# kunpengcompute/media

Measured on AMD Instinct MI355X. Metric: encoded fps @1080p I420 baseline-profile, 1/2/4/8 MI355X vs OpenH264 CPU, higher is better.
Workload: dtype u8

## Files before the change

### media_amd/csrc/k_me.h

```cpp
#pragma once
#include "dev_common.h"
#include "mc_filters.h"

namespace h264 {

enum { ME_R = 16, ME_AP = 4, ME_WS = 16 + 2 * ME_R + 2 * ME_AP, ME_WDW = ME_WS / 4, ME_GS = 18, ME_GP = 20, ME_PLS = ME_GS * ME_GP };

__device__ __forceinline__ void qpel_taps(int fx, int fy, int& o0, int& o1)
{
    const int PL = ME_PLS;
    const int G = 0, B = PL, H = 2 * PL, J = 3 * PL, R = 1, D = ME_GP;
    switch (fy * 4 + fx) {
        case 0: o0 = G; o1 = G; break;
        case 1: o0 = G; o1 = B; break;
        case 2: o0 = B; o1 = B; break;
        case 3: o0 = G + R; o1 = B; break;
        case 4: o0 = G; o1 = H; break;
        case 5: o0 = B; o1 = H; break;
        case 6: o0 = B; o1 = J; break;
        case 7: o0 = B; o1 = H + R; break;
        case 8: o0 = H; o1 = H; break;
        case 9: o0 = H; o1 = J; break;
        case 10: o0 = J; o1 = J; break;
        case 11: o0 = H + R; o1 = J; break;
        case 12: o0 = G + D; o1 = H; break;
        case 13: o0 = B + D; o1 = H; break;
        case 14: o0 = B + D; o1 = J; break;
        default: o0 = B + D; o1 = H + R; break;
    }
}


__device__ __forceinline__ uint32_t chroma_pred4(const uint8_t* cp, int cs2, int chh, int x0, int y0, int fx, int fy)
{
    const uint8_t* r0 = cp + (size_t)clip3(0, chh - 1, y0) * cs2;
    const uint8_t* r1 = cp + (size_t)clip3(0, chh - 1, y0 + 1) * cs2;
    uint32_t A, B, C, D;
    if (x0 >= 0 && (x0 & ~3) + 8 <= cs2) {
        const int xa = x0 & ~3, sh = x0 & 3;
        const uint32_t a0 = *(const uint32_t*)(r0 + xa), a1 = *(const uint32_t*)(r0 + xa + 4);
        const uint32_t c0 = *(const uint32_t*)(r1 + xa), c1 = *(const uint32_t*)(r1 + xa + 4);
        A = __builtin_amdgcn_alignbyte(a1, a0, sh); B = sh == 3 ? a1 : __builtin_amdgcn_alignbyte(a1, a0, sh + 1);
        C = __builtin_amdgcn_alignbyte(c1, c0, sh); D = sh == 3 ? c1 : __builtin_amdgcn_alignbyte(c1, c0, sh + 1);
    } else {
        A = B = C = D = 0;
#pragma unroll
        for (int k = 0; k < 4; k++) {
            const int xa = clip3(0, cs2 - 1, x0 + k), xb = clip3(0, cs2 - 1, x0 + k + 1);
            A |= (uint32_t)r0[xa] << (8 * k); B |= (uint32_t)r0[xb] << (8 * k);
            C |= (uint32_t)r1[xa] << (8 * k); D |= (uint32_t)r1[xb] << (8 * k);
        }
    }
    if ((fx | fy) == 0) return A;
    const int w00 = (8 - fx) * (8 - fy), w10 = fx * (8 - fy), w01 = (8 - fx) * fy, w11 = fx * fy;
    uint32_t o = 0;
#pragma unroll
    for (int k = 0; k < 4; k++)
        o |= (uint32_t)((w00 * byte_of(A, k) + w10 * byte_of(B, k) + w01 * byte_of(C, k) + w11 * byte_of(D, k) + 32) >> 6) << (8 * k);
    return o;
}

#ifndef ME_WAVES_MIN
#define ME_WAVES_MIN 6
#endif
template <bool IND = false>
__global__ __launch_bounds__(64) __attribute__((amdgpu_waves_per_eu(ME_WAVES_MIN, 8))) void k_me(FrameParams P0)
{
    if (AB_PRIO_ME) __builtin_amdgcn_s_setprio(AB_PRIO_ME);
    const FrameParams P = batch_view<IND>(P0, blockIdx.y);
    const int lane = threadIdx.x;
    const int mbi = P.band.row0 * P.mbw + xcd_mb_index(blockIdx.x, P.mbw * P.band.rows), my = P.mbdiv.row(mbi), mx = mbi - my * P.mbw;
    const int bx = 16 * mx, by = 16 * my;

    __shared__ __attribute__((aligned(16))) uint32_t s_win[ME_WS * ME_WDW];
    __shared__ __attribute__((aligned(16))) uint8_t s_src[256];
    __shared__ __attribute__((aligned(16))) uint8_t s_srcc[128];
    __shared__ __attribute__((aligned(16))) uint32_t s_ytab[32];
    __shared__ __attribute__((aligned(16))) uint8_t s_refc[128];
    enum { ME_B1_BYTES = (ME_GS + 5) * ME_GP * 2, ME_PL_BYTES = 4 * ME_PLS + 16 };
    enum { ME_TASKCAP = 760 };
    __shared__ __attribute__((aligned(16))) uint8_t s_scr[4 * ME_TASKCAP > ME_B1_BYTES + ME_PL_BYTES ? 4 * ME_TASKCAP : ME_B1_BYTES + ME_PL_BYTES];
    __shared__ unsigned s_ntask;
    uint32_t* const s_task = (uint32_t*)s_scr;
    int16_t* const s_b1 = (int16_t*)s_scr;
    uint8_t* const s_pl = s_scr + ME_B1_BYTES;

    const int pmw = __builtin_amdgcn_readfirstlane(P.rf == 0 ? *(const int*)(P.mb + mbi) : P.pmv[mbi]);
    if (P.rf == 0 && P.rf_last > 0 && lane == 0) P.pmv[mbi] = pmw;
    const int pmx = (int)(int16_t)(pmw & 0xFFFF), pmy = pmw >> 16;
    load_src_mb(P, mx, my, s_src, s_srcc, lane);
    const int rf = P.rf;
    unsigned prev_total = 0xFFFFFFFFu;
    if (rf > 0) {
        prev_total = (unsigned)__builtin_amdgcn_readfirstlane((int)P.me_total[mbi]);
        if (prev_total == 0u) return;
    }
    const uint8_t* const RY = P.ref[0];
    const uint8_t* const RU = P.ref[1];
    const uint8_t* const RV = P.ref[2];
    {
        const int wx0 = bx - ME_R - ME_AP, wy0 = by - ME_R - ME_AP;
        const bool inside = wx0 >= 0 && wx0 + 64 <= P.cw && wy0 >= 0 && wy0 + ME_WS <= P.ch;
        if (inside) {
            const int c = lane & 15, rg = lane >> 4;
            const uint8_t* rp = RY + (size_t)(wy0 + rg) * P.cw + wx0 + 4 * c;
            const size_t step = (size_t)4 * P.cw;
            uint32_t v[14];
#pragma unroll
            for (int t = 0; t < 14; t++) v[t] = *(const uint32_t*)(rp + t * step);
            if (c < ME_WDW)
#pragma unroll
                for (int t = 0; t < 14; t++) s_win[(rg + 4 * t) * ME_WDW + c] = v[t];
        } else {
            const bool interior = wx0 >= 0 && bx + 16 + ME_R + ME_AP <= P.cw;
            uint32_t v[13];
#pragma unroll
            for (int t = 0; t < 13; t++) {
                const int i = lane + 64 * t;
                const int row = i / ME_WDW, dw = i - row * ME_WDW;
                const int gy = clip3(0, P.ch - 1, wy0 + row);
                const int gx = wx0 + dw * 4;
                const uint8_t* rp = RY + (size_t)gy * P.cw;
                v[t] = 0;
                if (i < ME_WS * ME_WDW) {
                    if (interior) v[t] = *(const uint32_t*)(rp + gx);
                    else {
#pragma unroll
                        for (int k = 0; k < 4; k++) v[t] |= (uint32_t)rp[clip3(0, P.cw - 1, gx + k)] << (8 * k);
                    }
                }
            }
#pragma unroll
            for (int t = 0; t < 13; t++)
                if (lane + 64 * t < ME_WS * ME_WDW) s_win[lane + 64 * t] = v[t];
        }
    }
    if (rf == 0 && lane < 32) {
        const int pl = lane >> 4, row = (lane >> 1) & 7, xs = (lane & 1) * 4;
        *(uint32_t*)(s_refc + pl * 64 + row * 8 + xs) =
            *(const uint32_t*)((pl ? P.ref[2] : P.ref[1]) + (size_t)(8 * my + row) * (P.cw / 2) + 8 * mx + xs);
    }
    __syncthreads();
    const uint8_t* winb = (const uint8_t*)s_win;

    if (rf == 0) {
        typedef unsigned short pk16 __attribute__((ext_vector_type(2)));
        const int r = lane & 3, b4 = lane >> 2;
        const int cplz = lane >> 4, cyz = ((lane >> 3) & 1) * 4 + r, cxz = ((lane >> 2) & 1) * 4;
        const uint32_t sy = *(const uint32_t*)(s_src + ((b4 >> 2) * 4 + r) * 16 + (b4 & 3) * 4);
        const uint32_t sc = lane < 32 ? *(const uint32_t*)(s_srcc + cplz * 64 + cyz * 8 + cxz) : 0u;
        const uint32_t one = 0x00010001u;
        const pk16 sA = __builtin_bit_cast(pk16, (r & 1) ? 0xFFFFFFFFu : one);
        const pk16 mA = __builtin_bit_cast(pk16, r == 1 ? 2u * one : one);
        const pk16 mB = __builtin_bit_cast(pk16, r < 2 ? one : (r == 2 ? 0xFFFFFFFFu : 0xFFFEFFFEu));
        const uint32_t t0 = (uint32_t)(P.qy.thr_inter[0] - 1) | ((uint32_t)(P.qc.thr_inter[0] - 1) << 16);
        const uint32_t t1 = (uint32_t)(P.qy.thr_inter[1] - 1) | ((uint32_t)(P.qc.thr_inter[1] - 1) << 16);
        const uint32_t t2 = (uint32_t)(P.qy.thr_inter[2] - 1) | ((uint32_t)(P.qc.thr_inter[2] - 1) << 16);
        const pk16 th_even = __builtin_bit_cast(pk16, (r & 1) ? t2 : t0), th_odd = __builtin_bit_cast(pk16, (r & 1) ? t1 : t2);
        auto quantises_to_nothing = [&](uint32_t ry, uint32_t rc) -> bool {
            pk16 d[4];
#pragma unroll
            for (int k = 0; k < 4; k++) {
                const uint32_t sel = 0x0c040c00u + 0x00010001u * k;
                d[k] = __builtin_bit_cast(pk16, __builtin_amdgcn_perm(sc, sy, sel)) - __builtin_bit_cast(pk16, __builtin_amdgcn_perm(rc, ry, sel));
            }
            {
                const pk16 s0 = d[0] + d[3], s1 = d[1] + d[2], d0 = d[0] - d[3], d1 = d[1] - d[2];
                d[0] = s0 + s1; d[1] = d0 + d0 + d1; d[2] = s0 - s1; d[3] = d0 - d1 - d1;
            }
            uint32_t over = 0;
            int dc = 0;
#pragma unroll
            for (int c = 0; c < 4; c++) {
                if (c == 1 && __ballot(over != 0) != 0ull) return false;
                const pk16 q0 = __builtin_bit_cast(pk16, quad_bcast<0>(__builtin_bit_cast(int, d[c])));
                const pk16 q1 = __builtin_bit_cast(pk16, quad_bcast<1>(__builtin_bit_cast(int, d[c])));
                const pk16 q2 = __builtin_bit_cast(pk16, quad_bcast<2>(__builtin_bit_cast(int, d[c])));
                const pk16 q3 = __builtin_bit_cast(pk16, quad_bcast<3>(__builtin_bit_cast(int, d[c])));
                const pk16 A = q0 + sA * q3, B = q1 + sA * q2;
                const pk16 w = mA * A + mB * B;
                if (c == 0) dc = (int)(short)w.y;
                typedef short spk16 __attribute__((ext_vector_type(2)));
                const spk16 ws = __builtin_bit_cast(spk16, w);
                const pk16 aw = __builtin_bit_cast(pk16, __builtin_elementwise_max(ws, -ws));
                uint32_t ov = __builtin_bit_cast(uint32_t, __builtin_elementwise_sub_sat(aw, (c & 1) ? th_odd : th_even));
                if (c == 0 && r == 0) ov &= 0xFFFFu;
                over |= ov;
            }
            bool dcnz = false;
#pragma unroll
            for (int pl = 0; pl < 2; pl++) {
                const int d0 = __builtin_amdgcn_readlane(dc, pl * 16), d1 = __builtin_amdgcn_readlane(dc, pl * 16 + 4);
                const int d2 = __builtin_amdgcn_readlane(dc, pl * 16 + 8), d3 = __builtin_amdgcn_readlane(dc, pl * 16 + 12);
                const int t = P.qc.thr_dc_inter;
                dcnz |= iabs(d0 + d1 + d2 + d3) >= t || iabs(d0 - d1 + d2 - d3) >= t || iabs(d0 + d1 - d2 - d3) >= t || iabs(d0 - d1 - d2 + d3) >= t;
            }
            return !dcnz && __ballot(over != 0) == 0ull;
        };
        auto luma_sad = [&](uint32_t ry) -> unsigned {
            const int s = row_sum16_dpp((int)__builtin_amdgcn_sad_u8(sy, ry, 0u));
            return (unsigned)(__builtin_amdgcn_readlane(s, 0) + __builtin_amdgcn_readlane(s, 16) + __builtin_amdgcn_readlane(s, 32) + __builtin_amdgcn_readlane(s, 48));
        };
        auto settle = [&](int vx, int vy, uint32_t ry, uint32_t rc) {
            *(uint32_t*)(P.rec[0] + (size_t)(by + (b4 >> 2) * 4 + r) * P.cw + bx + (b4 & 3) * 4) = ry;
            if (lane < 32) *(uint32_t*)((cplz ? P.rec[2] : P.rec[1]) + (size_t)(8 * my + cyz) * (P.cw / 2) + 8 * mx + cxz) = rc;
            if (lane == 0) {
                uint4* m = (uint4*)(P.mb + mbi);
                m[0] = make_uint4(((uint32_t)vx & 0xFFFFu) | ((uint32_t)vy << 16), (uint32_t)MB_P16 | (0x80u << 8), 0u, 0u);
                m[1] = make_uint4(0u, 0u, 0u, 0u);
                const uint32_t v = ((uint32_t)vx & 0xFFFFu) | ((uint32_t)vy << 16);
                *(uint4*)(P.mvq + (size_t)mbi * 8) = make_uint4(v, v, v, v);
                P.me_cost[mbi] = 0;
                P.me_total[mbi] = 0u;
            }
        };
        {
            const uint32_t ry = s_win[(ME_R + ME_AP + (b4 >> 2) * 4 + r) * ME_WDW + (ME_R + ME_AP) / 4 + (b4 & 3)];
            const uint32_t rc = lane < 32 ? *(const uint32_t*)(s_refc + cplz * 64 + cyz * 8 + cxz) : 0u;
            if (luma_sad(ry) < (unsigned)P.sad_nz && quantises_to_nothing(ry, rc)) { settle(0, 0, ry, rc); return; }
        }
        const int rvx = ((pmx + 2) >> 2) * 4, rvy = ((pmy + 2) >> 2) * 4;
        if ((rvx | rvy) != 0) {
            const uint32_t ry = lds_ld4(winb, (ME_R + ME_AP + (b4 >> 2) * 4 + r + (rvy >> 2)) * ME_WS + ME_R + ME_AP + (b4 & 3) * 4 + (rvx >> 2));
            uint32_t rc = 0;
            if (lane < 32) rc = chroma_pred4(cplz ? P.ref[2] : P.ref[1], P.cw / 2, P.ch / 2, 8 * mx + cxz + (rvx >> 3), 8 * my + cyz + (rvy >> 3), rvx & 7, rvy & 7);
            if (luma_sad(ry) < (unsigned)P.sad_nz && quantises_to_nothing(ry, rc)) { settle(rvx, rvy, ry, rc); return; }
        }
    }

    unsigned best = 0xFFFFFFFFu;
    bool seeded = false;
    if (P.search == 1) {
        const int sx = (pmx + 2) >> 2, sy = (pmy + 2) >> 2;
        if (sx >= -ME_R && sx < ME_R && sy >= -ME_R && sy < ME_R) {
            const int g = lane >> 4, j = lane & 15;
            const int dyc = sy - 1 + (g < 3 ? g : 0);
            const uint4 sv = *(const uint4*)(s_src + 16 * j);
            const int ob = (ME_R + ME_AP + dyc + j) * ME_WS + ME_R + ME_AP + sx - 1;
            int sad3[3];
#pragma unroll
            for (int k = 0; k < 3; k++) {
                uint32_t a = __builtin_amdgcn_sad_u8(lds_ld4(winb, ob + k), sv.x, 0u);
                a = __builtin_amdgcn_sad_u8(lds_ld4(winb, ob + k + 4), sv.y, a);
                a = __builtin_amdgcn_sad_u8(lds_ld4(winb, ob + k + 8), sv.z, a);
                a = __builtin_amdgcn_sad_u8(lds_ld4(winb, ob + k + 12), sv.w, a);
                sad3[k] = row_sum16_dpp((int)a);
            }
            unsigned ckey = 0, nmin = 0xFFFFFFFFu;
#pragma unroll
            for (int gy = 0; gy < 3; gy++)
#pragma unroll
                for (int k = 0; k < 3; k++) {
                    const int dx = sx - 1 + k, dy = sy - 1 + gy;
                    const unsigned sad = (unsigned)__builtin_amdgcn_readlane(sad3[k], 16 * gy);
                    const unsigned key = ((sad + (unsigned)(P.lambda * (se_len(4 * dx - pmx) + se_len(4 * dy - pmy)))) << 10) | (unsigned)(((dy + ME_R) << 5) | (dx + ME_R));
                    const bool inr = dx >= -ME_R && dx < ME_R && dy >= -ME_R && dy < ME_R;
                    if (gy == 1 && k == 1) ckey = key;
                    else if (inr && key < nmin) nmin = key;
                }
            if (ckey < nmin) { best = ckey; seeded = true; }
        }
    }

    if (!seeded) {
        const int dxi = lane & 31, half = lane >> 5;
        const int col = dxi + ME_AP, cdw = col >> 2, sh = col & 3;
        if (lane < 32) s_ytab[lane] = ((uint32_t)__mul24(P.lambda, se_len(4 * (lane - ME_R) - pmy)) << 10) | ((uint32_t)lane << 5);
        uint32_t srow[16][4];
        const uint8_t* sp0 = P.src + (size_t)by * P.w + bx;
        if (bx + 16 <= P.w && by + 16 <= P.h && ((P.w | (int)(uintptr_t)P.src) & 3) == 0) {
#pragma unroll
            for (int j = 0; j < 16; j++) {
                typedef const __attribute__((address_space(4))) uint32_t* const_u32p;
                const const_u32p q = (const_u32p)(uintptr_t)(sp0 + (size_t)j * P.w);
                srow[j][0] = q[0]; srow[j][1] = q[1]; srow[j][2] = q[2]; srow[j][3] = q[3];
            }
        } else {
#pragma unroll
            for (int j = 0; j < 16; j++) {
                const uint4 v = *(const uint4*)(s_src + 16 * j);
                srow[j][0] = __builtin_amdgcn_readfirstlane(v.x); srow[j][1] = __builtin_amdgcn_readfirstlane(v.y);
                srow[j][2] = __builtin_amdgcn_readfirstlane(v.z); srow[j][3] = __builtin_amdgcn_readfirstlane(v.w);
            }
        }
        const uint32_t kbase = ((uint32_t)__mul24(P.lambda, se_len(4 * (dxi - ME_R) - pmx)) << 10) + (uint32_t)dxi;
        if (lane == 0) s_ntask = 0;
        lds_u32p wb0 = (lds_u32p)(s_win + (ME_AP + half * 16) * ME_WDW + cdw), wb1 = wb0 + 16 * ME_WDW;
        asm("" : "+v"(wb0));
        asm("" : "+v"(wb1));
        uint32_t acc[16];
#pragma unroll
        for (int kk = 0; kk < 16; kk++) acc[kk] = 0;
        uint32_t w[2][4];
#pragma unroll
        for (int c = 0; c < 4; c++) w[0][c] = wb0[c];
#pragma unroll
        for (int r = 0; r < 31; r++) {
            if (r + 1 < 31) {
#pragma unroll
                for (int c = 0; c < 4; c++) w[(r + 1) & 1][c] = r + 1 < 16 ? wb0[(r + 1) * ME_WDW + c] : wb1[(r + 1 - 16) * ME_WDW + c];
            }
            const uint32_t* wr = w[r & 1];
            const uint32_t a0 = __builtin_amdgcn_alignbyte(wr[1], wr[0], sh), a2 = __builtin_amdgcn_alignbyte(wr[3], wr[2], sh);
#pragma unroll
            for (int kk = 0; kk < 16; kk++) {
                const int j = r - kk;
                if (j >= 0 && j < 16) {
                    acc[kk] = __builtin_amdgcn_sad_u8(a0, srow[j][0], acc[kk]);
                    acc[kk] = __builtin_amdgcn_sad_u8(a2, srow[j][2], acc[kk]);
                }
            }
            __builtin_amdgcn_sched_barrier(0);
        }
        uint32_t lbk[16];
        uint32_t bestlb = 0xFFFFFFFFu;
#pragma unroll
        for (int q = 0; q < 4; q++) {
            const uint4 t = *(const uint4*)(s_ytab + half * 16 + 4 * q);
            lbk[4 * q] = (acc[4 * q] << 10) + (t.x + kbase); lbk[4 * q + 1] = (acc[4 * q + 1] << 10) + (t.y + kbase);
            lbk[4 * q + 2] = (acc[4 * q + 2] << 10) + (t.z + kbase); lbk[4 * q + 3] = (acc[4 * q + 3] << 10) + (t.w + kbase);
            bestlb = min(min(bestlb, lbk[4 * q]), min(lbk[4 * q + 1], min(lbk[4 * q + 2], lbk[4 * q + 3])));
        }
        bestlb = wave_min_u32_dpp(bestlb);
        auto rest_of_sad = [&](uint32_t key) -> uint32_t {
            const int ccol = (int)(key & 31) + ME_AP, csh = ccol & 3;
            lds_u32p p = (lds_u32p)(s_win + (ME_AP + (int)((key >> 5) & 31)) * ME_WDW + (ccol >> 2) + 1);
            asm("" : "+v"(p));
            uint32_t sum = 0;
            uint32_t v[2][4];
#pragma unroll
            for (int c = 0; c < 4; c++) v[0][c] = p[c];
#pragma unroll
            for (int j = 0; j < 16; j++) {
                if (j + 1 < 16) {
#pragma unroll
                    for (int c = 0; c < 4; c++) v[(j + 1) & 1][c] = p[(j + 1) * ME_WDW + c];
                }
                const uint32_t* vr = v[j & 1];
                sum = __builtin_amdgcn_sad_u8(__builtin_amdgcn_alignbyte(vr[1], vr[0], csh), srow[j][1], sum);
                sum = __builtin_amdgcn_sad_u8(__builtin_amdgcn_alignbyte(vr[3], vr[2], csh), srow[j][3], sum);
                asm volatile("" : "+v"(sum) : : "memory");
                __builtin_amdgcn_sched_barrier(0);
            }
            return sum;
        };
        uint32_t bound;
        {
            const int j = lane & 15, g = (lane >> 4) & 1;
            const int ccol = (int)(bestlb & 31) + ME_AP + 4 + 8 * g, crow = ME_AP + (int)((bestlb >> 5) & 31) + j;
            const uint32_t rv = lds_ld4(winb, crow * ME_WS + ccol), sv = *(const uint32_t*)(s_src + 16 * j + 4 + 8 * g);
            const int part = row_sum16_dpp(lane < 32 ? (int)__builtin_amdgcn_sad_u8(rv, sv, 0u) : 0);
            bound = bestlb + ((uint32_t)(__builtin_amdgcn_readlane(part, 0) + __builtin_amdgcn_readlane(part, 16)) << 10);
        }
        {
            unsigned n = 0;
#pragma unroll
            for (int kk = 0; kk < 16; kk++) n += lbk[kk] <= bound;
            unsigned at = n ? atomicAdd(&s_ntask, n) : 0u;
#pragma unroll
            for (int kk = 0; kk < 16; kk++)
                if (lbk[kk] <= bound) {
                    if (at < (unsigned)ME_TASKCAP) s_task[at] = lbk[kk];
                    at++;
                }
        }
        __syncthreads();
        const unsigned ntask = s_ntask;
        best = 0xFFFFFFFFu;
        if (ntask <= (unsigned)ME_TASKCAP) {
            for (unsigned t0 = 0; t0 < ntask; t0 += 64) {
                const bool on = t0 + lane < ntask;
                const uint32_t tk = s_task[on ? t0 + lane : 0];
                const uint32_t key = tk + (rest_of_sad(tk) << 10);
                best = on && key < best ? key : best;
            }
        } else {
#pragma unroll 1
            for (int kk = 0; kk < 16; kk++) {
                uint32_t tk = lbk[0];
#pragma unroll
                for (int i = 1; i < 16; i++) tk = kk == i ? lbk[i] : tk;
                const uint32_t key = tk + (rest_of_sad(tk) << 10);
                best = tk <= bound && key < best ? key : best;
            }
        }
        best = wave_min_u32_dpp(best);
        __syncthreads();
    }
    const int ix = (int)(best & 31) - ME_R, iy = (int)((best >> 5) & 31) - ME_R;

    const int oo = (iy + ME_R + ME_AP - 1) * ME_WS + ix + ME_R + ME_AP - 1;
    for (int i = lane; i < (ME_GS + 5) * 5; i += 64) {
        const int rr = i / 5, seg = (i - rr * 5) * 4;
        *(uint2*)(s_b1 + rr * ME_GP + seg) = htap4_pk(winb, oo + (rr - 2) * ME_WS + seg - 2);
    }
    __syncthreads();
    for (int i = lane; i < ME_GS * 5; i += 64) {
        const int y = i / 5, seg = (i - y * 5) * 4;
        const uint32_t Gv = lds_ld4(winb, oo + y * ME_WS + seg);
        uint2 rw[6];
#pragma unroll
        for (int k = 0; k < 6; k++) rw[k] = *(const uint2*)(s_b1 + (y + k) * ME_GP + seg);
        const uint32_t Bv = round5_pk(rw[2]);
        uint32_t Hv;
        {
            uint32_t c[6];
            const int o = oo + (y - 2) * ME_WS + seg;
            lds_u32p pc = (lds_u32p)(winb + (o & ~3));
            asm("" : "+v"(pc));
#pragma unroll
            for (int k = 0; k < 6; k++) c[k] = __builtin_amdgcn_alignbyte(pc[k * ME_WDW + 1], pc[k * ME_WDW], o & 3);
            Hv = round5_pk(vtap4_pk(c));
        }
        const uint32_t Jv = jtap4(rw);
        *(uint32_t*)(s_pl + y * ME_GP + seg) = Gv;
        *(uint32_t*)(s_pl + ME_PLS + y * ME_GP + seg) = Bv;
        *(uint32_t*)(s_pl + 2 * ME_PLS + y * ME_GP + seg) = Hv;
        *(uint32_t*)(s_pl + 3 * ME_PLS + y * ME_GP + seg) = Jv;
    }
    __syncthreads();

    const int cand = lane >> 3, bp = lane & 7, b4x = (bp & 3) * 4, b4y = (bp >> 2) * 4;
    typedef unsigned short pk16 __attribute__((ext_vector_type(2)));
    const uint32_t sel0 = 0x0c040c00u;
    pk16 S[16];
#pragma unroll
    for (int y = 0; y < 4; y++) {
        const uint32_t lo = *(const uint32_t*)(s_src + (b4y + y) * 16 + b4x), hi = *(const uint32_t*)(s_src + (b4y + 8 + y) * 16 + b4x);
#pragma unroll
        for (int x = 0; x < 4; x++) S[4 * y + x] = __builtin_bit_cast(pk16, __builtin_amdgcn_perm(hi, lo, sel0 + 0x00010001u * x));
    }
    S[0] = __builtin_bit_cast(pk16, __builtin_bit_cast(uint32_t, S[0]) ^ 0x80008000u);
    int cx = 4 * ix, cy = 4 * iy;
    unsigned centre_key;
    {
        const int r = lane & 3, b4 = lane >> 2;
        const uint32_t sy = *(const uint32_t*)(s_src + ((b4 >> 2) * 4 + r) * 16 + (b4 & 3) * 4);
        const uint32_t ry = lds_ld4(winb, (ME_R + ME_AP + (b4 >> 2) * 4 + r + iy) * ME_WS + ME_R + ME_AP + (b4 & 3) * 4 + ix);
        const int d0 = (int)(sy & 255u) - (int)(ry & 255u), d1 = (int)((sy >> 8) & 255u) - (int)((ry >> 8) & 255u);
        const int d2 = (int)((sy >> 16) & 255u) - (int)((ry >> 16) & 255u), d3 = (int)(sy >> 24) - (int)(ry >> 24);
        const int s0 = d0 + d3, s1 = d1 + d2, u0 = d0 - d3, u1 = d1 - d2;
        const int hr[4] = {s0 + s1, u0 + u1, s0 - s1, u0 - u1};
        const int sg1 = (lane & 1) ? -1 : 1, sg2 = (lane & 2) ? -1 : 1;
        int acc = 0;
#pragma unroll
        for (int c = 0; c < 4; c++) {
            const int y = __builtin_amdgcn_mov_dpp(hr[c], 0xB1, 0xf, 0xf, false) + sg1 * hr[c];
            const int z = __builtin_amdgcn_mov_dpp(y, 0x4E, 0xf, 0xf, false) + sg2 * y;
            acc += z < 0 ? -z : z;
        }
        const int s16 = row_sum16_dpp(acc);
        const int tot = __builtin_amdgcn_readlane(s16, 0) + __builtin_amdgcn_readlane(s16, 16) + __builtin_amdgcn_readlane(s16, 32) + __builtin_amdgcn_readlane(s16, 48);
        centre_key = ((unsigned)(tot >> 1) + (unsigned)(P.lambda * (se_len(cx - pmx) + se_len(cy - pmy)))) << 4;
    }
    unsigned best_cost_r = 0, bestk = 0xFFFFFFFFu;
#pragma unroll 1
    for (int round = 0; round < 2; round++) {
        const int step = round == 1 ? 1 : 2;
        const int ord = cand + 1;
        const int nn = cand >= 4 ? cand + 1 : cand;
        const int ddx = (nn % 3) - 1, ddy = (nn / 3) - 1;
        const int qx = cx + step * ddx, qy = cy + step * ddy;
        const int ox = qx - 4 * ix, oy = qy - 4 * iy;
        const int gx = 1 + (ox >> 2), gy = 1 + (oy >> 2);
        int t0, t1;
        qpel_taps(ox & 3, oy & 3, t0, t1);
        const int gb = (gy + b4y) * ME_GP + gx + b4x;
        lds_u32p pa = (lds_u32p)(s_pl + ((t0 + gb) & ~3));
        lds_u32p pb = (lds_u32p)(s_pl + ((t1 + gb) & ~3));
        asm("" : "+v"(pa));
        asm("" : "+v"(pb));
        const int sa = (t0 + gb) & 3, sb = (t1 + gb) & 3;
        pk16 d[16];
#pragma unroll
        for (int y = 0; y < 4; y++) {
            const int rl = (ME_GP / 4) * y, rh = (ME_GP / 4) * (y + 8);
            const uint32_t pl = avg4(__builtin_amdgcn_alignbyte(pa[rl + 1], pa[rl], sa), __builtin_amdgcn_alignbyte(pb[rl + 1], pb[rl], sb));
            const uint32_t ph = avg4(__builtin_amdgcn_alignbyte(pa[rh + 1], pa[rh], sa), __builtin_amdgcn_alignbyte(pb[rh + 1], pb[rh], sb));
#pragma unroll
            for (int x = 0; x < 4; x++)
                d[4 * y + x] = S[4 * y + x] - __builtin_bit_cast(pk16, __builtin_amdgcn_perm(ph, pl, sel0 + 0x00010001u * x));
        }
#pragma unroll
        for (int i = 0; i < 4; i++) {
            const pk16 s0 = d[4 * i] + d[4 * i + 3], s1 = d[4 * i + 1] + d[4 * i + 2];
            const pk16 d0 = d[4 * i] - d[4 * i + 3], d1 = d[4 * i + 1] - d[4 * i + 2];
            d[4 * i] = s0 + s1; d[4 * i + 1] = d0 + d1; d[4 * i + 2] = s0 - s1; d[4 * i + 3] = d0 - d1;
        }
        uint32_t sum = 0;
#pragma unroll
        for (int j = 0; j < 4; j++) {
            const pk16 s0 = d[j] + d[12 + j], s1 = d[4 + j] + d[8 + j];
            const pk16 d0 = d[j] - d[12 + j], d1 = d[4 + j] - d[8 + j];
            sum = __builtin_amdgcn_sad_u16(__builtin_bit_cast(uint32_t, s0 + s1), 0x80008000u, sum);
            sum = __builtin_amdgcn_sad_u16(__builtin_bit_cast(uint32_t, d0 + d1), 0x80008000u, sum);
            sum = __builtin_amdgcn_sad_u16(__builtin_bit_cast(uint32_t, s0 - s1), 0x80008000u, sum);
            sum = __builtin_amdgcn_sad_u16(__builtin_bit_cast(uint32_t, d0 - d1), 0x80008000u, sum);
        }
        const int s = group_sum8_dpp((int)sum);
        const unsigned cost = (unsigned)(s >> 1) + (unsigned)(P.lambda * (se_len(qx - pmx) + se_len(qy - pmy)));
        const unsigned key = (cost << 4) | (unsigned)ord;
        bestk = key < bestk ? key : bestk;
        if (round == 0) bestk = centre_key < bestk ? centre_key : bestk;
        bestk = wave_min_u32_dpp(bestk);
        const int w = (int)(bestk & 15);
        best_cost_r = bestk >> 4;
        if (w) {
            const int n = w - 1, wn = n >= 4 ? n + 1 : n;
            cx += step * ((wn % 3) - 1);
            cy += step * ((wn / 3) - 1);
        }
        bestk = best_cost_r << 4;
    }
    const int rbits = P.nref <= 1 ? 0 : (P.nref == 2 ? 1 : (rf == 0 ? 1 : 3));
    int shape = 0;
    int qvx0 = cx, qvy0 = cy, qvx1 = cx, qvy1 = cy, qvx2 = cx, qvy2 = cy, qvx3 = cx, qvy3 = cy;
    if (best_cost_r >= (unsigned)PART_TEST_MIN) {
        auto eval = [&](int qlx, int qly, int qhx, int qhy) -> uint32_t {
            const int oxl = qlx - 4 * ix, oyl = qly - 4 * iy, oxh = qhx - 4 * ix, oyh = qhy - 4 * iy;
            int t0, t1, u0, u1;
            qpel_taps(oxl & 3, oyl & 3, t0, t1);
            qpel_taps(oxh & 3, oyh & 3, u0, u1);
            const int gbl = (1 + (oyl >> 2) + b4y) * ME_GP + 1 + (oxl >> 2) + b4x;
            const int gbh = (1 + (oyh >> 2) + b4y + 8) * ME_GP + 1 + (oxh >> 2) + b4x;
            lds_u32p pal = (lds_u32p)(s_pl + ((t0 + gbl) & ~3)), pbl = (lds_u32p)(s_pl + ((t1 + gbl) & ~3));
            lds_u32p pah = (lds_u32p)(s_pl + ((u0 + gbh) & ~3)), pbh = (lds_u32p)(s_pl + ((u1 + gbh) & ~3));
            const int sal = (t0 + gbl) & 3, sbl = (t1 + gbl) & 3, sah = (u0 + gbh) & 3, sbh = (u1 + gbh) & 3;
            pk16 d[16];
#pragma unroll
            for (int y = 0; y < 4; y++) {
                const int r = (ME_GP / 4) * y;
                const uint32_t pl = avg4(__builtin_amdgcn_alignbyte(pal[r + 1], pal[r], sal), __builtin_amdgcn_alignbyte(pbl[r + 1], pbl[r], sbl));
                const uint32_t ph = avg4(__builtin_amdgcn_alignbyte(pah[r + 1], pah[r], sah), __builtin_amdgcn_alignbyte(pbh[r + 1], pbh[r], sbh));
#pragma unroll
                for (int x = 0; x < 4; x++)
                    d[4 * y + x] = S[4 * y + x] - __builtin_bit_cast(pk16, __builtin_amdgcn_perm(ph, pl, sel0 + 0x00010001u * x));
            }
#pragma unroll
            for (int i = 0; i < 4; i++) {
                const pk16 s0 = d[4 * i] + d[4 * i + 3], s1 = d[4 * i + 1] + d[4 * i + 2];
                const pk16 d0 = d[4 * i] - d[4 * i + 3], d1 = d[4 * i + 1] - d[4 * i + 2];
                d[4 * i] = s0 + s1; d[4 * i + 1] = d0 + d1; d[4 * i + 2] = s0 - s1; d[4 * i + 3] = d0 - d1;
            }
            typedef short spk16 __attribute__((ext_vector_type(2)));
            pk16 acc = {0, 0};
            auto add_abs = [&](pk16 v) {
                const spk16 t = __builtin_bit_cast(spk16, __builtin_bit_cast(uint32_t, v) ^ 0x80008000u);
                acc += __builtin_bit_cast(pk16, __builtin_elementwise_max(t, -t));
            };
#pragma unroll
            for (int j = 0; j < 4; j++) {
                const pk16 s0 = d[j] + d[12 + j], s1 = d[4 + j] + d[8 + j];
                const pk16 d0 = d[j] - d[12 + j], d1 = d[4 + j] - d[8 + j];
                add_abs(s0 + s1); add_abs(d0 + d1); add_abs(s0 - s1); add_abs(d0 - d1);
            }
            return __builtin_bit_cast(uint32_t, acc);
        };
        auto xor4 = [](int v) {
            int q = __builtin_amdgcn_update_dpp(0, v, 0x104, 0xf, 0x5, false);
            return __builtin_amdgcn_update_dpp(q, v, 0x114, 0xf, 0xa, false);
        };
        auto part_sums = [&](int sh, uint32_t acc, int& slo, int& shi) {
            const int alo = (int)(acc & 0xFFFFu), ahi = (int)(acc >> 16);
            if (sh == 1) { slo = group_sum8_dpp(alo); shi = group_sum8_dpp(ahi); }
            else if (sh == 2) {
                int v = alo + ahi;
                v += __builtin_amdgcn_mov_dpp(v, 0xB1, 0xf, 0xf, false);
                v += xor4(v);
                slo = v; shi = v;
            } else {
                int v = alo, u = ahi;
                v += __builtin_amdgcn_mov_dpp(v, 0xB1, 0xf, 0xf, false);
                u += __builtin_amdgcn_mov_dpp(u, 0xB1, 0xf, 0xf, false);
                slo = v + xor4(v); shi = u + xor4(u);
            }
        };
        auto min_over_candidates = [](unsigned k) {
            k = min(k, (unsigned)__shfl_xor((int)k, 8));
            k = min(k, (unsigned)__shfl_xor((int)k, 16));
            return min(k, (unsigned)__shfl_xor((int)k, 32));
        };
        const uint32_t acc0 = eval(4 * ix, 4 * iy, 4 * ix, 4 * iy);
        const int nn = cand >= 4 ? cand + 1 : cand, ddx = (nn % 3) - 1, ddy = (nn / 3) - 1;
        unsigned best_all = best_cost_r;
#pragma unroll 1
        for (int sh = 1; sh <= 3; sh++) {
            int clx = 4 * ix, cly = 4 * iy, chx = 4 * ix, chy = 4 * iy;
            unsigned klo, khi;
            {
                int slo, shi;
                part_sums(sh, acc0, slo, shi);
                const unsigned mvb = (unsigned)(P.lambda * (se_len(4 * ix - pmx) + se_len(4 * iy - pmy)));
                klo = ((unsigned)(slo >> 1) + mvb) << 4; khi = ((unsigned)(shi >> 1) + mvb) << 4;
            }
#pragma unroll 1
            for (int round = 0; round < 2; round++) {
                const int step = round == 1 ? 1 : 2;
                const int qlx = clx + step * ddx, qly = cly + step * ddy, qhx = chx + step * ddx, qhy = chy + step * ddy;
                int slo, shi;
                part_sums(sh, eval(qlx, qly, qhx, qhy), slo, shi);
                const unsigned cl = (unsigned)(slo >> 1) + (unsigned)(P.lambda * (se_len(qlx - pmx) + se_len(qly - pmy)));
                const unsigned chh = (unsigned)(shi >> 1) + (unsigned)(P.lambda * (se_len(qhx - pmx) + se_len(qhy - pmy)));
                klo = min_over_candidates(min(klo, (cl << 4) | (unsigned)(cand + 1)));
                khi = min_over_candidates(min(khi, (chh << 4) | (unsigned)(cand + 1)));
                const int wl = (int)(klo & 15u), wh = (int)(khi & 15u);
                if (wl) { const int n = wl - 1, wn = n >= 4 ? n + 1 : n; clx += step * ((wn % 3) - 1); cly += step * ((wn / 3) - 1); }
                if (wh) { const int n = wh - 1, wn = n >= 4 ? n + 1 : n; chx += step * ((wn % 3) - 1); chy += step * ((wn / 3) - 1); }
                klo &= ~15u; khi &= ~15u;
            }
            const unsigned l0 = (unsigned)__builtin_amdgcn_readlane((int)klo, 0) >> 4, l2 = (unsigned)__builtin_amdgcn_readlane((int)klo, 2) >> 4;
            const unsigned h0 = (unsigned)__builtin_amdgcn_readlane((int)khi, 0) >> 4, h2 = (unsigned)__builtin_amdgcn_readlane((int)khi, 2) >> 4;
            const unsigned tot = (sh == 1 ? l0 + h0 : (sh == 2 ? l0 + l2 : l0 + l2 + h0 + h2)) + (unsigned)(P.lambda * (sh == 3 ? 8 + 3 * rbits : 2 + rbits));
            if (tot < best_all) {
                best_all = tot; shape = sh;
                qvx0 = __builtin_amdgcn_readlane(clx, 0); qvy0 = __builtin_amdgcn_readlane(cly, 0);
                qvx1 = __builtin_amdgcn_readlane(clx, 2); qvy1 = __builtin_amdgcn_readlane(cly, 2);
                qvx2 = __builtin_amdgcn_readlane(chx, 0); qvy2 = __builtin_amdgcn_readlane(chy, 0);
                qvx3 = __builtin_amdgcn_readlane(chx, 2); qvy3 = __builtin_amdgcn_readlane(chy, 2);
            }
        }
        best_cost_r = best_all;
    }
    const unsigned total = best_cost_r + (unsigned)(P.lambda * rbits);
    const bool better = total < prev_total;
    if (better) {
        const int y = lane >> 2, seg = (lane & 3) * 4;
        const int pl = lane >> 4, cyy = (lane >> 1) & 7, cxx = (lane & 1) * 4;
        if (shape == 0) {
            const int ox = cx - 4 * ix, oy = cy - 4 * iy;
            int t0, t1;
            qpel_taps(ox & 3, oy & 3, t0, t1);
            const int gb = (1 + (oy >> 2) + y) * ME_GP + 1 + (ox >> 2) + seg;
            *(uint32_t*)(P.rec[0] + (size_t)(by + y) * P.cw + bx + seg) = avg4(lds_ld4(s_pl, t0 + gb), lds_ld4(s_pl, t1 + gb));
            if (lane < 32)
                *(uint32_t*)((pl ? P.rec[2] : P.rec[1]) + (size_t)(8 * my + cyy) * (P.cw / 2) + 8 * mx + cxx) =
                    chroma_pred4(pl ? RV : RU, P.cw / 2, P.ch / 2, 8 * mx + cxx + (cx >> 3), 8 * my + cyy + (cy >> 3), cx & 7, cy & 7);
        } else {
            {
                const bool lowq = y < 8, leftq = seg < 8;
                const int vx = lowq ? (leftq ? qvx0 : qvx1) : (leftq ? qvx2 : qvx3), vy = lowq ? (leftq ? qvy0 : qvy1) : (leftq ? qvy2 : qvy3);
                const int ox = vx - 4 * ix, oy = vy - 4 * iy;
                int t0, t1;
                qpel_taps(ox & 3, oy & 3, t0, t1);
                const int gb = (1 + (oy >> 2) + y) * ME_GP + 1 + (ox >> 2) + seg;
                *(uint32_t*)(P.rec[0] + (size_t)(by + y) * P.cw + bx + seg) = avg4(lds_ld4(s_pl, t0 + gb), lds_ld4(s_pl, t1 + gb));
            }
            if (lane < 32) {
                const bool lowq = cyy < 4, leftq = cxx < 4;
                const int vx = lowq ? (leftq ? qvx0 : qvx1) : (leftq ? qvx2 : qvx3), vy = lowq ? (leftq ? qvy0 : qvy1) : (leftq ? qvy2 : qvy3);
                *(uint32_t*)((pl ? P.rec[2] : P.rec[1]) + (size_t)(8 * my + cyy) * (P.cw / 2) + 8 * mx + cxx) =
                    chroma_pred4(pl ? RV : RU, P.cw / 2, P.ch / 2, 8 * mx + cxx + (vx >> 3), 8 * my + cyy + (vy >> 3), vx & 7, vy & 7);
            }
        }
        if (lane == 0) {
            uint4* m = (uint4*)(P.mb + mbi);
            const uint32_t type = shape ? (uint32_t)(MB_P16X8 + shape - 1) : (uint32_t)MB_P16;
            auto pk = [](int x, int yv) { return ((uint32_t)x & 0xFFFFu) | ((uint32_t)yv << 16); };
            m[0] = make_uint4(pk(qvx0, qvy0), type | ((uint32_t)rf << 16), 0u, 0u);
            m[1] = make_uint4(0u, 0u, 0u, 0u);
            *(uint4*)(P.mvq + (size_t)mbi * 8) = make_uint4(pk(qvx0, qvy0), pk(qvx1, qvy1), pk(qvx2, qvy2), pk(qvx3, qvy3));
            P.me_total[mbi] = total;
        }
    }
    const unsigned best_cost = better ? total : prev_total;
    if (lane == 0) P.me_cost[mbi] = (uint16_t)(best_cost < 16383u ? best_cost : 16383u);
    if (rf != P.rf_last) return;
    if (best_cost >= (unsigned)INTRA_TEST_MIN) {
        const bool topav = P.sl.has_top(my), leftav = mx > 0;
        uint8_t* const s_nb = (uint8_t*)s_ytab;
        int nb = 0;
        if (lane < 16) nb = topav ? src_px(P.src, P.w, P.h, bx + lane, by - 1) : 0;
        else if (lane < 32) nb = leftav ? src_px(P.src, P.w, P.h, bx - 1, by + lane - 16) : 0;
        if (lane < 32) s_nb[lane] = (uint8_t)nb;
        const int s16 = row_sum16_dpp(lane < 32 ? nb : 0);
        const int st = __builtin_amdgcn_readlane(s16, 0), sl = __builtin_amdgcn_readlane(s16, 16);
        const int dc = (topav && leftav) ? (st + sl + 16) >> 5 : topav ? (st + 8) >> 4 : leftav ? (sl + 8) >> 4 : 128;
        __syncthreads();
        const int mode = lane >> 4, blk = lane & 15, x0 = (blk & 3) * 4, y0 = (blk >> 2) * 4;
        int d[16];
#pragma unroll
        for (int y = 0; y < 4; y++) {
            const uint32_t sw = *(const uint32_t*)(s_src + (y0 + y) * 16 + x0);
#pragma unroll
            for (int x = 0; x < 4; x++) {
                const int pr = mode == 0 ? s_nb[x0 + x] : mode == 1 ? s_nb[16 + y0 + y] : dc;
                d[4 * y + x] = (int)((sw >> (8 * x)) & 255u) - pr;
            }
        }
        const int satd = row_sum16_dpp(lane < 48 ? hadamard_abs(d) : 0) >> 1;
        const bool ok = mode == 0 ? topav : mode == 1 ? leftav : mode == 2;
        const unsigned est = wave_min_u32_dpp(ok ? (unsigned)satd : 0xFFFFFFFFu) + 8u * (unsigned)P.lambda;
        if (est < best_cost) {
            if (lane == 0) {
                uint4* m = (uint4*)(P.mb + mbi);
                m[0] = make_uint4(0u, (uint32_t)MB_I16, 0u, 0u);
                m[1] = make_uint4(0u, 0u, 0u, 0u);
                P.me_cost[mbi] = (uint16_t)(0x8000u | (best_cost < 16383u ? best_cost : 16383u));
                *P.anyintra = P.pic_serial;
            }
            return;
        }
    }
}

}
```

Measured before the change: 26220.

## Restructure sub-pel refinement: table taps, paired-row plane build, specialized half-pel round

The quarter-pel tap switch becomes a constexpr table copied into LDS and indexed per lane. The half-pel plane build now has each lane produce two rows, reusing the overlapping 6-tap window, and divide-by-5 is replaced with a multiply-shift. The half-pel round is specialised: each candidate reads a single plane at a fixed offset with no averaging. The aim is to cut divergent switch code, redundant LDS loads and arithmetic in motion estimation. It also adds an optional compile-time A/B repeat macro for profiling phases, which is disabled by default.

Result: faster. 26600 (median of 6 runs) (+1.4%).

```diff
diff --git a/media_amd/csrc/k_me.h b/media_amd/csrc/k_me.h
--- a/media_amd/csrc/k_me.h
+++ b/media_amd/csrc/k_me.h
@@ -6,29 +6,60 @@
 
 enum { ME_R = 16, ME_AP = 4, ME_WS = 16 + 2 * ME_R + 2 * ME_AP, ME_WDW = ME_WS / 4, ME_GS = 18, ME_GP = 20, ME_PLS = ME_GS * ME_GP };
 
-__device__ __forceinline__ void qpel_taps(int fx, int fy, int& o0, int& o1)
+struct QpelTap { int o0, o1; };
+constexpr QpelTap qpel_tap(int i)
 {
     const int PL = ME_PLS;
     const int G = 0, B = PL, H = 2 * PL, J = 3 * PL, R = 1, D = ME_GP;
-    switch (fy * 4 + fx) {
-        case 0: o0 = G; o1 = G; break;
-        case 1: o0 = G; o1 = B; break;
-        case 2: o0 = B; o1 = B; break;
-        case 3: o0 = G + R; o1 = B; break;
-        case 4: o0 = G; o1 = H; break;
-        case 5: o0 = B; o1 = H; break;
-        case 6: o0 = B; o1 = J; break;
-        case 7: o0 = B; o1 = H + R; break;
-        case 8: o0 = H; o1 = H; break;
-        case 9: o0 = H; o1 = J; break;
-        case 10: o0 = J; o1 = J; break;
-        case 11: o0 = H + R; o1 = J; break;
-        case 12: o0 = G + D; o1 = H; break;
-        case 13: o0 = B + D; o1 = H; break;
-        case 14: o0 = B + D; o1 = J; break;
-        default: o0 = B + D; o1 = H + R; break;
+    switch (i) {
+        case 0: return {G, G};
+        case 1: return {G, B};
+        case 2: return {B, B};
+        case 3: return {G + R, B};
+        case 4: return {G, H};
+        case 5: return {B, H};
+        case 6: return {B, J};
+        case 7: return {B, H + R};
+        case 8: return {H, H};
+        case 9: return {H, J};
+        case 10: return {J, J};
+        case 11: return {H + R, J};
+        case 12: return {G + D, H};
+        case 13: return {B + D, H};
+        case 14: return {B + D, J};
+        default: return {B + D, H + R};
     }
 }
+__device__ __forceinline__ void qpel_taps(int fx, int fy, int& o0, int& o1)
+{
+    const QpelTap t = qpel_tap(fy * 4 + fx);
+    o0 = t.o0; o1 = t.o1;
+}
+#define ME_QT(i) ((uint32_t)qpel_tap(i).o0 | ((uint32_t)qpel_tap(i).o1 << 16))
+__constant__ const uint32_t c_qpel_tap[16] = {ME_QT(0), ME_QT(1), ME_QT(2), ME_QT(3), ME_QT(4), ME_QT(5), ME_QT(6), ME_QT(7),
+                                              ME_QT(8), ME_QT(9), ME_QT(10), ME_QT(11), ME_QT(12), ME_QT(13), ME_QT(14), ME_QT(15)};
+#undef ME_QT
+__device__ __forceinline__ void qpel_taps_lds(const uint32_t* s_tap, int ox, int oy, int& o0, int& o1)
+{
+    const uint32_t t = s_tap[((oy & 3) << 2) | (ox & 3)];
+    o0 = (int)(t & 0xFFFFu); o1 = (int)(t >> 16);
+}
+
+#ifndef ME_AB_REPEAT
+#define ME_AB_REPEAT 0
+#endif
+#if ME_AB_REPEAT
+__device__ __forceinline__ int me_ab_reps(int bit)
+{
+    int n = ((ME_AB_REPEAT >> bit) & 1) ? 2 : 1;
+    asm volatile("" : "+s"(n));
+    return n;
+}
+__device__ __forceinline__ int me_ab_next() { asm volatile("" ::: "memory"); return 1; }
+#define ME_AB_PHASE(bit) for (int ab_n = me_ab_reps(bit), ab_i = 0; ab_i < ab_n; ab_i += me_ab_next())
+#else
+#define ME_AB_PHASE(bit) if constexpr (true)
+#endif
 
 
 __device__ __forceinline__ uint32_t chroma_pred4(const uint8_t* cp, int cs2, int chh, int x0, int y0, int fx, int fy)
@@ -390,35 +421,38 @@
     const int ix = (int)(best & 31) - ME_R, iy = (int)((best >> 5) & 31) - ME_R;
 
     const int oo = (iy + ME_R + ME_AP - 1) * ME_WS + ix + ME_R + ME_AP - 1;
+    uint32_t* const s_tap = s_ytab;
+    if (lane < 16) s_tap[lane] = c_qpel_tap[lane];
+    ME_AB_PHASE(0) {
     for (int i = lane; i < (ME_GS + 5) * 5; i += 64) {
-        const int rr = i / 5, seg = (i - rr * 5) * 4;
+        const int rr = (i * 205) >> 10, seg = (i - rr * 5) * 4;
         *(uint2*)(s_b1 + rr * ME_GP + seg) = htap4_pk(winb, oo + (rr - 2) * ME_WS + seg - 2);
     }
     __syncthreads();
-    for (int i = lane; i < ME_GS * 5; i += 64) {
-        const int y = i / 5, seg = (i - y * 5) * 4;
-        const uint32_t Gv = lds_ld4(winb, oo + y * ME_WS + seg);
-        uint2 rw[6];
-#pragma unroll
-        for (int k = 0; k < 6; k++) rw[k] = *(const uint2*)(s_b1 + (y + k) * ME_GP + seg);
-        const uint32_t Bv = round5_pk(rw[2]);
-        uint32_t Hv;
+    if (lane < (ME_GS / 2) * 5) {
+        const int yp = (lane * 205) >> 10, seg = (lane - yp * 5) * 4, y0 = 2 * yp;
+        uint2 rw[7];
+#pragma unroll
+        for (int k = 0; k < 7; k++) rw[k] = *(const uint2*)(s_b1 + (y0 + k) * ME_GP + seg);
+        uint32_t c[7];
         {
-            uint32_t c[6];
-            const int o = oo + (y - 2) * ME_WS + seg;
+            const int o = oo + (y0 - 2) * ME_WS + seg;
             lds_u32p pc = (lds_u32p)(winb + (o & ~3));
             asm("" : "+v"(pc));
 #pragma unroll
-            for (int k = 0; k < 6; k++) c[k] = __builtin_amdgcn_alignbyte(pc[k * ME_WDW + 1], pc[k * ME_WDW], o & 3);
-            Hv = round5_pk(vtap4_pk(c));
-        }
-        const uint32_t Jv = jtap4(rw);
-        *(uint32_t*)(s_pl + y * ME_GP + seg) = Gv;
-        *(uint32_t*)(s_pl + ME_PLS + y * ME_GP + seg) = Bv;
-        *(uint32_t*)(s_pl + 2 * ME_PLS + y * ME_GP + seg) = Hv;
-        *(uint32_t*)(s_pl + 3 * ME_PLS + y * ME_GP + seg) = Jv;
+            for (int k = 0; k < 7; k++) c[k] = __builtin_amdgcn_alignbyte(pc[k * ME_WDW + 1], pc[k * ME_WDW], o & 3);
+        }
+#pragma unroll
+        for (int r = 0; r < 2; r++) {
+            uint8_t* const q = s_pl + (y0 + r) * ME_GP + seg;
+            *(uint32_t*)q = c[2 + r];
+            *(uint32_t*)(q + ME_PLS) = round5_pk(rw[2 + r]);
+            *(uint32_t*)(q + 2 * ME_PLS) = round5_pk(vtap4_pk(c + r));
+            *(uint32_t*)(q + 3 * ME_PLS) = jtap4(rw + r);
+        }
     }
     __syncthreads();
+    }
 
     const int cand = lane >> 3, bp = lane & 7, b4x = (bp & 3) * 4, b4y = (bp >> 2) * 4;
     typedef unsigned short pk16 __attribute__((ext_vector_type(2)));
@@ -433,7 +467,7 @@
     S[0] = __builtin_bit_cast(pk16, __builtin_bit_cast(uint32_t, S[0]) ^ 0x80008000u);
     int cx = 4 * ix, cy = 4 * iy;
     unsigned centre_key;
-    {
+    ME_AB_PHASE(1) {
         const int r = lane & 3, b4 = lane >> 2;
         const uint32_t sy = *(const uint32_t*)(s_src + ((b4 >> 2) * 4 + r) * 16 + (b4 & 3) * 4);
         const uint32_t ry = lds_ld4(winb, (ME_R + ME_AP + (b4 >> 2) * 4 + r + iy) * ME_WS + ME_R + ME_AP + (b4 & 3) * 4 + ix);
@@ -453,34 +487,15 @@
         const int tot = __builtin_amdgcn_readlane(s16, 0) + __builtin_amdgcn_readlane(s16, 16) + __builtin_amdgcn_readlane(s16, 32) + __builtin_amdgcn_readlane(s16, 48);
         centre_key = ((unsigned)(tot >> 1) + (unsigned)(P.lambda * (se_len(cx - pmx) + se_len(cy - pmy)))) << 4;
     }
-    unsigned best_cost_r = 0, bestk = 0xFFFFFFFFu;
-#pragma unroll 1
-    for (int round = 0; round < 2; round++) {
-        const int step = round == 1 ? 1 : 2;
-        const int ord = cand + 1;
-        const int nn = cand >= 4 ? cand + 1 : cand;
-        const int ddx = (nn % 3) - 1, ddy = (nn / 3) - 1;
-        const int qx = cx + step * ddx, qy = cy + step * ddy;
-        const int ox = qx - 4 * ix, oy = qy - 4 * iy;
-        const int gx = 1 + (ox >> 2), gy = 1 + (oy >> 2);
-        int t0, t1;
-        qpel_taps(ox & 3, oy & 3, t0, t1);
-        const int gb = (gy + b4y) * ME_GP + gx + b4x;
-        lds_u32p pa = (lds_u32p)(s_pl + ((t0 + gb) & ~3));
-        lds_u32p pb = (lds_u32p)(s_pl + ((t1 + gb) & ~3));
-        asm("" : "+v"(pa));
-        asm("" : "+v"(pb));
-        const int sa = (t0 + gb) & 3, sb = (t1 + gb) & 3;
+    const int nn = cand >= 4 ? cand + 1 : cand;
+    const int ddx = (nn % 3) - 1, ddy = (nn / 3) - 1;
+    auto satd8 = [&](const uint32_t pl[4], const uint32_t ph[4]) -> int {
         pk16 d[16];
 #pragma unroll
-        for (int y = 0; y < 4; y++) {
-            const int rl = (ME_GP / 4) * y, rh = (ME_GP / 4) * (y + 8);
-            const uint32_t pl = avg4(__builtin_amdgcn_alignbyte(pa[rl + 1], pa[rl], sa), __builtin_amdgcn_alignbyte(pb[rl + 1], pb[rl], sb));
-            const uint32_t ph = avg4(__builtin_amdgcn_alignbyte(pa[rh + 1], pa[rh], sa), __builtin_amdgcn_alignbyte(pb[rh + 1], pb[rh], sb));
+        for (int y = 0; y < 4; y++)
 #pragma unroll
             for (int x = 0; x < 4; x++)
-                d[4 * y + x] = S[4 * y + x] - __builtin_bit_cast(pk16, __builtin_amdgcn_perm(ph, pl, sel0 + 0x00010001u * x));
-        }
+                d[4 * y + x] = S[4 * y + x] - __builtin_bit_cast(pk16, __builtin_amdgcn_perm(ph[y], pl[y], sel0 + 0x00010001u * x));
 #pragma unroll
         for (int i = 0; i < 4; i++) {
             const pk16 s0 = d[4 * i] + d[4 * i + 3], s1 = d[4 * i + 1] + d[4 * i + 2];
@@ -497,20 +512,64 @@
             sum = __builtin_amdgcn_sad_u16(__builtin_bit_cast(uint32_t, s0 - s1), 0x80008000u, sum);
             sum = __builtin_amdgcn_sad_u16(__builtin_bit_cast(uint32_t, d0 - d1), 0x80008000u, sum);
         }
-        const int s = group_sum8_dpp((int)sum);
-        const unsigned cost = (unsigned)(s >> 1) + (unsigned)(P.lambda * (se_len(qx - pmx) + se_len(qy - pmy)));
-        const unsigned key = (cost << 4) | (unsigned)ord;
-        bestk = key < bestk ? key : bestk;
-        if (round == 0) bestk = centre_key < bestk ? centre_key : bestk;
-        bestk = wave_min_u32_dpp(bestk);
+        return group_sum8_dpp((int)sum);
+    };
+    auto mv_rate = [&](int step) -> unsigned {
+        return (unsigned)(P.lambda * (se_len(cx + step * ddx - pmx) + se_len(cy + step * ddy - pmy)));
+    };
+    auto take_winner = [&](unsigned key, unsigned stay, int step) -> unsigned {
+        const unsigned bestk = wave_min_u32_dpp(key < stay ? key : stay);
         const int w = (int)(bestk & 15);
-        best_cost_r = bestk >> 4;
         if (w) {
             const int n = w - 1, wn = n >= 4 ? n + 1 : n;
             cx += step * ((wn % 3) - 1);
             cy += step * ((wn / 3) - 1);
         }
-        bestk = best_cost_r << 4;
+        return bestk >> 4;
+    };
+    unsigned best_cost_r;
+    {
+        int s;
+        ME_AB_PHASE(2) {
+            const int go = ME_PLS * ((ddx != 0) + 2 * (ddy != 0)) + ((ddy >= 0) + b4y) * ME_GP + (ddx >= 0) + b4x;
+            lds_u32p pa = (lds_u32p)(s_pl + (go & ~3));
+            asm("" : "+v"(pa));
+            const int sa = go & 3;
+            uint32_t pl[4], ph[4];
+#pragma unroll
+            for (int y = 0; y < 4; y++) {
+                const int rl = (ME_GP / 4) * y, rh = (ME_GP / 4) * (y + 8);
+                pl[y] = __builtin_amdgcn_alignbyte(pa[rl + 1], pa[rl], sa);
+                ph[y] = __builtin_amdgcn_alignbyte(pa[rh + 1], pa[rh], sa);
+            }
+            s = satd8(pl, ph);
+        }
+        const unsigned cost = (unsigned)(s >> 1) + mv_rate(2);
+        best_cost_r = take_winner((cost << 4) | (unsigned)(cand + 1), centre_key, 2);
+    }
+    {
+        int s;
+        ME_AB_PHASE(3) {
+            const int ox = cx + ddx - 4 * ix, oy = cy + ddy - 4 * iy;
+            int t0, t1;
+            qpel_taps_lds(s_tap, ox, oy, t0, t1);
+            const int gb = (1 + (oy >> 2) + b4y) * ME_GP + 1 + (ox >> 2) + b4x;
+            lds_u32p pa = (lds_u32p)(s_pl + ((t0 + gb) & ~3));
+            lds_u32p pb = (lds_u32p)(s_pl + ((t1 + gb) & ~3));
+            asm("" : "+v"(pa));
+            asm("" : "+v"(pb));
+            const int sa = (t0 + gb) & 3, sb = (t1 + gb) & 3;
+            uint32_t pl[4], ph[4];
+#pragma unroll
+            for (int y = 0; y < 4; y++) {
+                const int rl = (ME_GP / 4) * y, rh = (ME_GP / 4) * (y + 8);
+                pl[y] = avg4(__builtin_amdgcn_alignbyte(pa[rl + 1], pa[rl], sa), __builtin_amdgcn_alignbyte(pb[rl + 1], pb[rl], sb));
+                ph[y] = avg4(__builtin_amdgcn_alignbyte(pa[rh + 1], pa[rh], sa), __builtin_amdgcn_alignbyte(pb[rh + 1], pb[rh], sb));
+            }
+            s = satd8(pl, ph);
+        }
+        const unsigned cost = (unsigned)(s >> 1) + mv_rate(1);
+        best_cost_r = take_winner((cost << 4) | (unsigned)(cand + 1), best_cost_r << 4, 1);
     }
     const int rbits = P.nref <= 1 ? 0 : (P.nref == 2 ? 1 : (rf == 0 ? 1 : 3));
     int shape = 0;
@@ -519,8 +578,8 @@
         auto eval = [&](int qlx, int qly, int qhx, int qhy) -> uint32_t {
             const int oxl = qlx - 4 * ix, oyl = qly - 4 * iy, oxh = qhx - 4 * ix, oyh = qhy - 4 * iy;
             int t0, t1, u0, u1;
-            qpel_taps(oxl & 3, oyl & 3, t0, t1);
-            qpel_taps(oxh & 3, oyh & 3, u0, u1);
+            qpel_taps_lds(s_tap, oxl, oyl, t0, t1);
+            qpel_taps_lds(s_tap, oxh, oyh, u0, u1);
             const int gbl = (1 + (oyl >> 2) + b4y) * ME_GP + 1 + (oxl >> 2) + b4x;
             const int gbh = (1 + (oyh >> 2) + b4y + 8) * ME_GP + 1 + (oxh >> 2) + b4x;
             lds_u32p pal = (lds_u32p)(s_pl + ((t0 + gbl) & ~3)), pbl = (lds_u32p)(s_pl + ((t1 + gbl) & ~3));
@@ -581,7 +640,6 @@
             return min(k, (unsigned)__shfl_xor((int)k, 32));
         };
         const uint32_t acc0 = eval(4 * ix, 4 * iy, 4 * ix, 4 * iy);
-        const int nn = cand >= 4 ? cand + 1 : cand, ddx = (nn % 3) - 1, ddy = (nn / 3) - 1;
         unsigned best_all = best_cost_r;
 #pragma unroll 1
         for (int sh = 1; sh <= 3; sh++) {
@@ -623,9 +681,11 @@
     }
     const unsigned total = best_cost_r + (unsigned)(P.lambda * rbits);
     const bool better = total < prev_total;
-    if (better) {
-        const int y = lane >> 2, seg = (lane & 3) * 4;
-        const int pl = lane >> 4, cyy = (lane >> 1) & 7, cxx = (lane & 1) * 4;
+    if (better) ME_AB_PHASE(4) {
+        int wl = lane;
+        asm volatile("" : "+v"(wl));
+        const int y = wl >> 2, seg = (wl & 3) * 4;
+        const int pl = wl >> 4, cyy = (wl >> 1) & 7, cxx = (wl & 1) * 4;
         if (shape == 0) {
             const int ox = cx - 4 * ix, oy = cy - 4 * iy;
             int t0, t1;
@@ -641,7 +701,7 @@
                 const int vx = lowq ? (leftq ? qvx0 : qvx1) : (leftq ? qvx2 : qvx3), vy = lowq ? (leftq ? qvy0 : qvy1) : (leftq ? qvy2 : qvy3);
                 const int ox = vx - 4 * ix, oy = vy - 4 * iy;
                 int t0, t1;
-                qpel_taps(ox & 3, oy & 3, t0, t1);
+                qpel_taps_lds(s_tap, ox, oy, t0, t1);
                 const int gb = (1 + (oy >> 2) + y) * ME_GP + 1 + (ox >> 2) + seg;
                 *(uint32_t*)(P.rec[0] + (size_t)(by + y) * P.cw + bx + seg) = avg4(lds_ld4(s_pl, t0 + gb), lds_ld4(s_pl, t1 + gb));
             }
```
